# heliaxdev/kzg-setup-powersoftau

Measured on NVIDIA B200. Metric: G1+G2 points/sec parse+decompress+subgroup-check+ark re-encode (2^21 compressed G1 + 2^21 compressed G2 per step), higher is better.
Workload: dtype u32 limbs (12x32-bit Montgomery, IMAD.WIDE carry chains)

## Files before the change

### kzg_setup_powersoftau_b200/csrc/capi.cu

```cuda
#include <cuda_runtime.h>
#include <stdint.h>
#include <stdio.h>
#include <string.h>

#include <chrono>
#include <string>
#include <vector>

#include "../../include/ptau_b200.h"
#include <future>

#include "context.h"
#include "kernels.h"

using ptau::GpuSlot;
using ptau::kBufs;
using ptau::kMaxGpus;

namespace {

constexpr size_t kEdgePoints = 148 * 2 * 128;

#define CUDA_TRY(ctx, expr)                                                          \
  do {                                                                               \
// ... 320 lines not shown
        npts = rem < chunk ? rem : chunk;
      else if (rem > 2 * kEdgePoints)
        npts = rem - kEdgePoints;
      else
        npts = rem < chunk ? rem : chunk;
      if (r.issued >= kBufs) {
        CUDA_TRY(ctx, cudaEventSynchronize(s.ev_k1[b]));
        float ms = 0;
        CUDA_TRY(ctx, cudaEventElapsedTime(&ms, s.ev_k0[b], s.ev_k1[b]));
        tm.kernel_ms[g] += ms;
      }
      const uint8_t* src = (const uint8_t*)in + r.next * (size_t)ri;
      uint8_t* dst = out ? (uint8_t*)out + r.next * (size_t)ro : nullptr;
      CUDA_TRY(ctx, cudaMemcpyAsync(s.d_in[b], src, npts * ri, cudaMemcpyHostToDevice, s.stream[b]));
      CUDA_TRY(ctx, cudaEventRecord(s.ev_k0[b], s.stream[b]));
      CUDA_TRY(ctx, ptau::launch_convert(group, in_fmt, out_fmt, s.d_in[b], s.d_out[b], npts, checks, r.next,
                                         s.d_status, s.stream[b]));
      CUDA_TRY(ctx, cudaEventRecord(s.ev_k1[b], s.stream[b]));
      if (out) {
        CUDA_TRY(ctx, cudaMemcpyAsync(dst, s.d_out[b], npts * ro, cudaMemcpyDeviceToHost, s.stream[b]));
        tm.d2h_bytes[g] += npts * ro;
      }
      tm.h2d_bytes[g] += npts * ri;
      tm.kernel_launches++;
      r.next += npts;
      r.issued++;
      more = true;
    }
  }
  unsigned long long status = PTAU_STATUS_NONE;
  for (int g = 0; g < G; g++) {
    GpuSlot& s = ctx->gpu[g];
    CUDA_TRY(ctx, cudaSetDevice(s.device));
    CUDA_TRY(ctx, cudaEventRecord(s.ev_last, s.stream[1]));
    CUDA_TRY(ctx, cudaStreamWaitEvent(s.stream[0], s.ev_last, 0));
    unsigned long long st = PTAU_STATUS_NONE;
    CUDA_TRY(ctx, cudaMemcpyAsync(&st, s.d_status, sizeof(st), cudaMemcpyDeviceToHost, s.stream[0]));
    CUDA_TRY(ctx, cudaEventRecord(s.ev_last, s.stream[0]));
    CUDA_TRY(ctx, cudaStreamSynchronize(s.stream[0]));
    CUDA_TRY(ctx, cudaStreamSynchronize(s.stream[1]));
    if (st < status) status = st;
    float ms = 0;
    CUDA_TRY(ctx, cudaEventElapsedTime(&ms, s.ev_first, s.ev_last));
    tm.gpu_ms[g] = ms;
    int pending = rg[g].issued < kBufs ? rg[g].issued : kBufs;
    for (int b = 0; b < pending; b++) {
      float k = 0;
// ... 671 lines not shown
```

### kzg_setup_powersoftau_b200/csrc/consts.inc

```
PTAU_HD Fq k_b1_mont() {
  const uint32_t c[12] = {0x000cfff3u, 0xaa270000u, 0xfc34000au, 0x53cc0032u, 0x6b0a807fu, 0x478fe97au, 0xe6ba24d7u, 0xb1d37ebeu, 0xbf78ab2fu, 0x8ec9733bu, 0x3d83de7eu, 0x09d64551u};
  Fq r;
#pragma unroll
  for (int i = 0; i < 12; i++) r.l[i] = c[i];
  return r;
}
PTAU_HD Fq k_beta_mont() {
  const uint32_t c[12] = {0x798a64e8u, 0x30f1361bu, 0x7ece5a2au, 0xf3b8ddabu, 0xc61577f7u, 0x16a8ca3au, 0x74fd029bu, 0xc26a2ff8u, 0x60701c6eu, 0x3636b766u, 0x241b6160u, 0x051ba4abu};
  Fq r;
#pragma unroll
  for (int i = 0; i < 12; i++) r.l[i] = c[i];
  return r;
}
PTAU_HD Fq k_psi_cx1_mont() {
  const uint32_t c[12] = {0x867545c3u, 0x890dc9e4u, 0x3285a5d5u, 0x2af32253u, 0x309b7e2cu, 0x50880866u, 0x7e881024u, 0xa20d1b8cu, 0xe2db9068u, 0x14e4f04fu, 0x1564853au, 0x14e56d3fu};
  Fq r;
#pragma unroll
  for (int i = 0; i < 12; i++) r.l[i] = c[i];
  return r;
}
PTAU_HD Fq k_psi_cy0_mont() {
  const uint32_t c[12] = {0xa55c9ad1u, 0x3e2f585du, 0x86c18183u, 0x4294213du, 0x8b623732u, 0x382844c8u, 0x19103e18u, 0x92ad2afdu, 0xac7cf0b9u, 0x1d794e4fu, 0x7d825ec8u, 0x0bd592fcu};
  Fq r;
#pragma unroll
// ... 85 lines not shown
  return r;
}
PTAU_HD Fq k_frob12_c0_mont() {
  const uint32_t c[12] = {0xb319d465u, 0x07089552u, 0xb50a8313u, 0xc6695f92u, 0xd117228fu, 0x97e83cccu, 0xb2dc29eeu, 0xa35baecau, 0x5daace4du, 0x1ce393eau, 0xb0fb66ebu, 0x08f2220fu};
  Fq r;
#pragma unroll
  for (int i = 0; i < 12; i++) r.l[i] = c[i];
  return r;
}
PTAU_HD Fq k_frob12_c1_mont() {
  const uint32_t c[12] = {0x4ce5d646u, 0xb2f66aadu, 0xfc497cecu, 0x5842a06bu, 0x2599d394u, 0xcf4895d4u, 0x40a8e8d0u, 0xc11b9cbau, 0xe5a0de89u, 0x2e3813cbu, 0x88847fafu, 0x110eefdau};
  Fq r;
#pragma unroll
  for (int i = 0; i < 12; i++) r.l[i] = c[i];
  return r;
}
PTAU_HD Fq k_pm1_half_plain() {
  const uint32_t c[12] = {0xffffd555u, 0xdcff7fffu, 0x58a9ffffu, 0x0f55ffffu, 0x7b587b12u, 0xb3986950u, 0x79c2895fu, 0xb23ba5c2u, 0x21a5d66bu, 0x258dd3dbu, 0x1cbff34du, 0x0d0088f5u};
  Fq r;
#pragma unroll
  for (int i = 0; i < 12; i++) r.l[i] = c[i];
  return r;
}
#define PTAU_P34_STEPS 80
#define PTAU_P34_CHAIN_INIT {0x4d, 0x91, 0x41, 0x7f, 0x45, 0x67, 0x6b, 0x4f, 0x4f, 0x6d, 0x6d, 0x69, 0x33, 0x7d, 0x4d, 0x6f, 0x5d, 0x49, 0x8d, 0x6b, 0x35, 0x33, 0x6d, 0x47, 0x33, 0x31, 0x67, 0x47, 0x59, 0x47, 0x89, 0x37, 0x57, 0x75, 0x79, 0x5b, 0x4f, 0x33, 0x57, 0x43, 0x8d, 0x55, 0x21, 0x9f, 0x5d, 0x33, 0x8f, 0x33, 0x79, 0x9f, 0x45, 0x5b, 0x4f, 0x4f, 0x4f, 0x37, 0x5b, 0x65, 0x59, 0x4f, 0x4f, 0x4f, 0x4f, 0x4d, 0x23, 0x6f, 0x4f, 0x5f, 0x4f, 0x4f, 0x4f, 0x4f, 0x4f, 0x4f, 0x4f, 0x35, 0x45, 0x45, 0x21, 0x10}
```

### kzg_setup_powersoftau_b200/csrc/kernels.cu

```cuda
#include <cuda_runtime.h>
#include <stdint.h>
#include <string.h>

#include <type_traits>

#include "kernels.h"
#include "point.cuh"
#include "msm.cuh"

namespace ptau {

#ifndef PTAU_BLOCK
#define PTAU_BLOCK 128
#endif
#ifndef PTAU_MINBLOCKS_G1
#define PTAU_MINBLOCKS_G1 2
#endif
#ifndef PTAU_MINBLOCKS_G2
#define PTAU_MINBLOCKS_G2 2
#endif
#ifndef PTAU_BLOCK_G1
#define PTAU_BLOCK_G1 PTAU_BLOCK
#endif
#ifndef PTAU_BLOCK_G2
// ... 49 lines not shown
  }
}

template <int BLK>
__device__ __forceinline__ void stage_out_flat(uint32_t* __restrict__ g, const uint32_t* sm, int nwords) {
  int nvec = nwords >> 2;
  uint4* g4 = reinterpret_cast<uint4*>(g);
  const uint4* s4 = reinterpret_cast<const uint4*>(sm);
  for (int i = threadIdx.x; i < nvec; i += BLK) g4[i] = s4[i];
  for (int i = (nvec << 2) + threadIdx.x; i < nwords; i += BLK) g[i] = sm[i];
}

template <int G, int INFMT, int OUTFMT, bool HEAVY>
constexpr int convert_smem_words() {
  constexpr int BLK = G == PTAU_G1 ? PTAU_BLOCK_G1 : PTAU_BLOCK_G2;
  constexpr int SIN = smem_stride(record_bytes(G, INFMT) / 4);
  constexpr int SOUT = smem_stride(record_bytes(G, OUTFMT) / 4);
  return BLK * (SIN > SOUT ? SIN : SOUT) + ((G == PTAU_G2 && HEAVY) ? BLK * PTAU_PARK_WORDS : 0);
}

#ifndef PTAU_MINBLOCKS_LIGHT
#define PTAU_MINBLOCKS_LIGHT 2
#endif
template <int G, int INFMT, int OUTFMT, bool HEAVY>
__global__ void __launch_bounds__((G == PTAU_G1 ? PTAU_BLOCK_G1 : PTAU_BLOCK_G2),
                                  (!HEAVY ? PTAU_MINBLOCKS_LIGHT : G == PTAU_G1 ? PTAU_MINBLOCKS_G1 : PTAU_MINBLOCKS_G2))
    convert_kernel(const uint32_t* __restrict__ in, uint32_t* __restrict__ out, uint64_t n, uint32_t checks,
                   uint64_t base_index, unsigned long long* __restrict__ status) {
  constexpr int BLK = G == PTAU_G1 ? PTAU_BLOCK_G1 : PTAU_BLOCK_G2;
  constexpr int WIN = record_bytes(G, INFMT) / 4;
  constexpr int WOUT = record_bytes(G, OUTFMT) / 4;
  constexpr int SIN = smem_stride(WIN), SOUT = smem_stride(WOUT);
  constexpr int SMAX = SIN > SOUT ? SIN : SOUT;
  extern __shared__ __align__(16) uint32_t sm[];

  const uint64_t rec0 = (uint64_t)blockIdx.x * BLK;
  const int nrec = (int)((n - rec0) < (uint64_t)BLK ? (n - rec0) : (uint64_t)BLK);
  const int tid = threadIdx.x;

  stage_in<BLK, WIN, SIN>(in + rec0 * WIN, sm, nrec);
  __syncthreads();

  uint32_t win[WIN];
  if (tid < nrec) {
    if (WIN % 4 == 0) {
      const uint4* s4 = reinterpret_cast<const uint4*>(sm + tid * SIN);
#pragma unroll
      for (int j = 0; j < WIN / 4; j++) {
        uint4 v = s4[j];
        win[4 * j] = v.x;
        win[4 * j + 1] = v.y;
        win[4 * j + 2] = v.z;
        win[4 * j + 3] = v.w;
      }
    } else {
      const uint2* s2 = reinterpret_cast<const uint2*>(sm + tid * SIN);
#pragma unroll
      for (int j = 0; j < WIN / 2; j++) {
        uint2 v = s2[j];
        win[2 * j] = v.x;
        win[2 * j + 1] = v.y;
      }
    }
  }
  __syncthreads();

  if (tid < nrec) {
    uint32_t st;
    if (G == PTAU_G2 && HEAVY) {
      Park<BLK> pk;
      pk.base = (uint32_t)__cvta_generic_to_shared(sm + BLK * SMAX + tid);
      st = g2_process<INFMT, HEAVY, BLK>(win, OUTFMT, sm + tid * SOUT, checks, pk);
    } else {
      uint32_t wout[WOUT];
      if (G == PTAU_G2) {
        Park<BLK> pk;
        pk.base = 0;
        st = g2_process<INFMT, HEAVY, BLK>(win, OUTFMT, wout, checks, pk);
      } else {
        st = g1_process<INFMT, HEAVY>(win, OUTFMT, wout, checks);
      }
      if (WOUT % 4 == 0) {
        uint4* s4 = reinterpret_cast<uint4*>(sm + tid * SOUT);
#pragma unroll
        for (int j = 0; j < WOUT / 4; j++) s4[j] = make_uint4(wout[4 * j], wout[4 * j + 1], wout[4 * j + 2], wout[4 * j + 3]);
      } else {
        uint2* s2 = reinterpret_cast<uint2*>(sm + tid * SOUT);
#pragma unroll
        for (int j = 0; j < WOUT / 2; j++) s2[j] = make_uint2(wout[2 * j], wout[2 * j + 1]);
      }
    }
    if (st != PTAU_OK) atomicMin(status, (unsigned long long)(((base_index + rec0 + tid) << 8) | st));
  }
  __syncthreads();
  stage_out<BLK, WOUT, SOUT>(out + rec0 * WOUT, sm, nrec);
}

template <int G, int INFMT, int OUTFMT, bool HEAVY>
static cudaError_t launch_inst(const void* d_in, void* d_out, uint64_t n, uint32_t checks, uint64_t base_index,
                               unsigned long long* d_status, cudaStream_t stream) {
  constexpr int BLK = G == PTAU_G1 ? PTAU_BLOCK_G1 : PTAU_BLOCK_G2;
  constexpr int SMEM = convert_smem_words<G, INFMT, OUTFMT, HEAVY>() * 4;
  auto kern = convert_kernel<G, INFMT, OUTFMT, HEAVY>;
  if (SMEM > 48 * 1024) {
    cudaError_t e = cudaFuncSetAttribute(kern, cudaFuncAttributeMaxDynamicSharedMemorySize, SMEM);
    if (e != cudaSuccess) return e;
  }
  unsigned grid = (unsigned)((n + BLK - 1) / BLK);
  kern<<<grid, BLK, SMEM, stream>>>((const uint32_t*)d_in, (uint32_t*)d_out, n, checks, base_index, d_status);
  return cudaGetLastError();
}

template <int G, int INFMT, int OUTFMT>
static cudaError_t launch_one(const void* d_in, void* d_out, uint64_t n, uint32_t checks, uint64_t base_index,
                              unsigned long long* d_status, cudaStream_t stream) {
  if (n == 0) return cudaSuccess;
  const bool light = INFMT == PTAU_FMT_ZCASH_COMPRESSED
                         ? !(checks & PTAU_CHECK_SUBGROUP)
                         : !(checks & (PTAU_CHECK_ON_CURVE | PTAU_CHECK_SUBGROUP));
  if (light) return launch_inst<G, INFMT, OUTFMT, false>(d_in, d_out, n, checks, base_index, d_status, stream);
  return launch_inst<G, INFMT, OUTFMT, true>(d_in, d_out, n, checks, base_index, d_status, stream);
}

template <int G, int INFMT>
static cudaError_t launch_in(int out_fmt, const void* d_in, void* d_out, uint64_t n, uint32_t checks,
                             uint64_t base_index, unsigned long long* d_status, cudaStream_t stream) {
  switch (out_fmt) {
    case PTAU_FMT_ZCASH_UNCOMPRESSED:
      return launch_one<G, INFMT, PTAU_FMT_ZCASH_UNCOMPRESSED>(d_in, d_out, n, checks, base_index, d_status, stream);
    case PTAU_FMT_ARK_UNCOMPRESSED:
      return launch_one<G, INFMT, PTAU_FMT_ARK_UNCOMPRESSED>(d_in, d_out, n, checks, base_index, d_status, stream);
    case PTAU_FMT_ARK_MONT_LIMBS:
      return launch_one<G, INFMT, PTAU_FMT_ARK_MONT_LIMBS>(d_in, d_out, n, checks, base_index, d_status, stream);
  }
  return cudaErrorInvalidValue;
}

template <int G>
static cudaError_t launch_g(int in_fmt, int out_fmt, const void* d_in, void* d_out, uint64_t n, uint32_t checks,
                            uint64_t base_index, unsigned long long* d_status, cudaStream_t stream) {
  switch (in_fmt) {
    case PTAU_FMT_ZCASH_UNCOMPRESSED:
      return launch_in<G, PTAU_FMT_ZCASH_UNCOMPRESSED>(out_fmt, d_in, d_out, n, checks, base_index, d_status, stream);
    case PTAU_FMT_ZCASH_COMPRESSED:
// ... 899 lines not shown
```

### kzg_setup_powersoftau_b200/csrc/kernels.h

```cpp
#pragma once
#include <cuda_runtime.h>
#include <stdint.h>

namespace ptau {

struct MsmGeom;

cudaError_t launch_convert(int group, int in_fmt, int out_fmt, const void* d_in, void* d_out, uint64_t n,
                           uint32_t checks, uint64_t base_index, unsigned long long* d_status,
                           cudaStream_t stream);

cudaError_t launch_generate(int group, int fmt, const uint32_t* d_scalars, void* d_out, uint64_t n,
                            cudaStream_t stream);

cudaError_t launch_generate_win(int group, int fmt, const uint32_t* s0_mont, const uint32_t (*pw_mont)[8],
                                const uint32_t* d_tbl, void* d_out, uint64_t first, uint64_t n, cudaStream_t stream);

struct MsmPlan {
  int c, W, a, lgL;
  uint32_t NB;
  uint64_t buckets, segments;
  uint64_t off_counts, off_offsets, off_cursor, off_entries, off_buckets, off_segments, off_wsum, off_order, scratch_bytes;
};
void msm_g1_plan(uint64_t n, MsmPlan* plan);
cudaError_t launch_msm_g1(const void* d_pts, const void* d_scalars, uint64_t n, void* d_scratch, void* d_out,
                          int* launches, cudaStream_t stream);
void msm_g2_plan(uint64_t n, MsmPlan* plan);
cudaError_t launch_msm_g2(const void* d_pts, const void* d_scalars, uint64_t n, void* d_scratch, void* d_out,
                          int* launches, cudaStream_t stream);
cudaError_t launch_msm_g2_sums(const uint32_t* pts, const uint32_t* entries, const uint32_t* offsets, const uint32_t* order,
                               uint32_t m, uint32_t* buckets, const MsmGeom& g, uint32_t nseg, uint32_t* segs, uint32_t* wsum,
                               uint32_t* out, cudaStream_t stream);

// ... 17 lines not shown
```

### kzg_setup_powersoftau_b200/csrc/point.cuh

```cuda
#pragma once
#include "curve.cuh"
#include "../../include/ptau_b200.h"

namespace ptau {

PTAU_HD uint32_t bswap32(uint32_t v) {
#ifdef __CUDA_ARCH__
  return __byte_perm(v, 0, 0x0123);
#else
  return (v >> 24) | ((v >> 8) & 0xff00u) | ((v << 8) & 0xff0000u) | (v << 24);
#endif
}

PTAU_HD Fq fq_from_be_words(const uint32_t* w) {
  Fq r;
#pragma unroll
  for (int j = 0; j < 12; j++) r.l[j] = bswap32(w[11 - j]);
  return r;
}
PTAU_HD void fq_to_be_words(const Fq& a, uint32_t* w) {
#pragma unroll
  for (int j = 0; j < 12; j++) w[11 - j] = bswap32(a.l[j]);
}
PTAU_HD Fq fq_from_le_words(const uint32_t* w) {
  Fq r;
#pragma unroll
  for (int j = 0; j < 12; j++) r.l[j] = w[j];
  return r;
}
PTAU_HD void fq_to_le_words(const Fq& a, uint32_t* w) {
#pragma unroll
  for (int j = 0; j < 12; j++) w[j] = a.l[j];
}

#ifdef __CUDACC__
__constant__ uint8_t K_P34_CHAIN_D[PTAU_P34_STEPS] = PTAU_P34_CHAIN_INIT;
#endif
static const uint8_t K_P34_CHAIN_H[PTAU_P34_STEPS] = PTAU_P34_CHAIN_INIT;

PTAU_HD_NOINLINE Fq fq_pow_p34(const Fq& a) {
#ifdef __CUDA_ARCH__
  const uint8_t* chain = K_P34_CHAIN_D;
#else
  const uint8_t* chain = K_P34_CHAIN_H;
#endif
  Fq tbl[8];
  tbl[0] = a;
  Fq a2 = fq_sqr(a);
#pragma unroll 1
  for (int i = 1; i < 8; i++) tbl[i] = fq_mul(tbl[i - 1], a2);
  Fq acc = tbl[(chain[0] & 15) >> 1];
#pragma unroll 1
  for (int s = 1; s < PTAU_P34_STEPS; s++) {
    int c = chain[s];
    int n = c >> 4;
#if defined(__CUDA_ARCH__) && !defined(PTAU_POW_CALLS)
#pragma unroll 1
    for (int k = 0; k < n; k++) acc = fq_sqr_inl(acc);
#else
#pragma unroll 1
    for (int k = 0; k < n; k++) acc = fq_sqr(acc);
#endif
    if (c & 15) acc = fq_mul(acc, tbl[(c & 15) >> 1]);
  }
  return acc;
}

PTAU_HD Fq fq_sqrt(const Fq& a, bool& ok) {
  Fq s = fq_mul(fq_pow_p34(a), a);
  ok = fq_eq(fq_sqr(s), a);
  return s;
}

PTAU_HD_NOINLINE Fq2 fq2_sqrt(const Fq2& a, bool& ok) {
  Fq n = fq_add(fq_sqr(a.c0), fq_sqr(a.c1));
  Fq s = fq_mul(fq_pow_p34(n), n);
  Fq half = k_half_mont();
  Fq d = fq_mul(fq_add(a.c0, s), half);
  if (fq_is_zero(d)) d = fq_mul(fq_sub(a.c0, s), half);
  Fq t = fq_pow_p34(d);
  Fq x0 = fq_mul(d, t);
  Fq chi = fq_mul(x0, t);
  Fq w = fq_mul(fq_mul(a.c1, t), half);
  bool qr = fq_eq(chi, fq_one()) || fq_is_zero(d);
  Fq2 r;
  Fq nx0 = fq_neg(x0);
// ... 8 lines not shown

PTAU_HD bool fq_plain_is_largest(const Fq& yp) { return fq_gt_plain(yp, k_pm1_half_plain()); }

PTAU_HD Fq fq_plain_neg(const Fq& a) {
  const uint32_t pl[12] = PTAU_P_LIMBS;
  Fq r;
  uint32_t bf = 0;
  bool z = fq_is_zero(a);
#pragma unroll
  for (int i = 0; i < 12; i++) {
    uint64_t t = (uint64_t)pl[i] - a.l[i] - bf;
    bf = (uint32_t)(t >> 63);
    r.l[i] = z ? 0u : (uint32_t)t;
  }
  return r;
}

PTAU_HD constexpr int record_bytes(int group, int fmt) {
  return fmt == PTAU_FMT_ZCASH_COMPRESSED    ? (group == PTAU_G1 ? 48 : 96)
         : fmt == PTAU_FMT_ARK_MONT_LIMBS    ? (group == PTAU_G1 ? 104 : 200)
                                             : (group == PTAU_G1 ? 96 : 192);
}

template <int INFMT, bool HEAVY = true>
PTAU_HD uint32_t g1_process(const uint32_t* in, int out_fmt, uint32_t* out, uint32_t checks) {
  if (!HEAVY) checks &= PTAU_CHECK_REJECT_INFINITY;
  Fq xp, yp, xm, ym;
  uint32_t st = PTAU_OK;
  bool inf = false;
  bool have_mont = false;

  if (INFMT == PTAU_FMT_ZCASH_COMPRESSED) {
    xp = fq_from_be_words(in);
    uint32_t fl = xp.l[11] >> 29;
    xp.l[11] &= 0x1fffffffu;
    bool greatest = fl & 1u;
    yp = fq_zero();
    if (!(fl & 4u)) {
      st = PTAU_BAD_FLAGS;
    } else if (fl & 2u) {
      if ((fl & 1u) || !fq_is_zero(xp)) st = PTAU_BAD_FLAGS;
      inf = true;
      yp.l[0] = 1;
    } else if (fq_plain_ge_p(xp)) {
      st = PTAU_BAD_NON_CANONICAL;
    }
    if (st == PTAU_OK && !inf) {
      xm = fq_to_mont(xp);
      Fq rhs = fq_add(fq_mul(fq_sqr(xm), xm), k_b1_mont());
      bool ok;
      ym = fq_sqrt(rhs, ok);
      if (!ok) st = PTAU_BAD_NOT_ON_CURVE;
      yp = fq_from_mont(ym);
      if (fq_plain_is_largest(yp) != greatest) {
        ym = fq_neg(ym);
        yp = fq_plain_neg(yp);
      }
      have_mont = true;
    }
  } else if (INFMT == PTAU_FMT_ARK_MONT_LIMBS) {
    xm = fq_from_le_words(in);
    ym = fq_from_le_words(in + 12);
    inf = (in[24] & 0xffu) != 0;
    if (fq_plain_ge_p(xm) || fq_plain_ge_p(ym)) {
      st = PTAU_BAD_NON_CANONICAL;
      xm = fq_zero();
      ym = fq_zero();
    }
    have_mont = true;
    xp = fq_from_mont(xm);
    yp = fq_from_mont(ym);
    if (HEAVY && st == PTAU_OK && !inf && (checks & PTAU_CHECK_ON_CURVE) && !g1_on_curve(xm, ym)) st = PTAU_BAD_NOT_ON_CURVE;
  } else {
    if (INFMT == PTAU_FMT_ZCASH_UNCOMPRESSED) {
      xp = fq_from_be_words(in);
      yp = fq_from_be_words(in + 12);
    } else {
      xp = fq_from_le_words(in);
      yp = fq_from_le_words(in + 12);
    }
// ... 31 lines not shown
      out[0] = 0x40u;
    } else {
      fq_to_be_words(xp, out);
      fq_to_be_words(yp, out + 12);
    }
  } else {
    if (st == PTAU_OK && !have_mont) {
      xm = fq_to_mont(xp);
      ym = fq_to_mont(yp);
      have_mont = true;
    }
    if (!have_mont) {
      xm = fq_zero();
      ym = fq_zero();
    }
    fq_to_le_words(xm, out);
    fq_to_le_words(ym, out + 12);
    out[24] = inf ? 1u : 0u;
    out[25] = 0;
  }
  return st;
}

template <int INFMT, bool HEAVY, int PSTRIDE>
PTAU_HD uint32_t g2_process(const uint32_t* in, int out_fmt, uint32_t* out, uint32_t checks, Park<PSTRIDE> pk) {
  if (!HEAVY) checks &= PTAU_CHECK_REJECT_INFINITY;
  Fq2 xp, yp, xm, ym;
  uint32_t st = PTAU_OK;
  bool inf = false;
  bool have_mont = false;
  bool off_curve = false;

  if (INFMT == PTAU_FMT_ZCASH_COMPRESSED) {
    xp.c1 = fq_from_be_words(in);
    xp.c0 = fq_from_be_words(in + 12);
    uint32_t fl = xp.c1.l[11] >> 29;
    xp.c1.l[11] &= 0x1fffffffu;
    bool greatest = fl & 1u;
    yp = fq2_zero();
    if (!(fl & 4u)) {
      st = PTAU_BAD_FLAGS;
    } else if (fl & 2u) {
      if ((fl & 1u) || !fq2_is_zero(xp)) st = PTAU_BAD_FLAGS;
      inf = true;
      yp.c0.l[0] = 1;
    } else if (fq_plain_ge_p(xp.c1) || fq_plain_ge_p(xp.c0)) {
      st = PTAU_BAD_NON_CANONICAL;
    }
    if (st == PTAU_OK && !inf) {
      xm.c0 = fq_to_mont(xp.c0);
      xm.c1 = fq_to_mont(xp.c1);
      Fq2 b;
      b.c0 = k_b1_mont();
      b.c1 = b.c0;
      Fq2 rhs = fq2_add(fq2_mul(fq2_sqr(xm), xm), b);
      bool ok;
      ym = fq2_sqrt(rhs, ok);
      if (!ok) st = PTAU_BAD_NOT_ON_CURVE;
      yp.c0 = fq_from_mont(ym.c0);
      yp.c1 = fq_from_mont(ym.c1);
      bool largest = fq_is_zero(yp.c1) ? fq_plain_is_largest(yp.c0) : fq_plain_is_largest(yp.c1);
      if (largest != greatest) {
        ym = fq2_neg(ym);
        yp.c0 = fq_plain_neg(yp.c0);
        yp.c1 = fq_plain_neg(yp.c1);
      }
      have_mont = true;
    }
  } else if (INFMT == PTAU_FMT_ARK_MONT_LIMBS) {
    xm.c0 = fq_from_le_words(in);
    xm.c1 = fq_from_le_words(in + 12);
    ym.c0 = fq_from_le_words(in + 24);
    ym.c1 = fq_from_le_words(in + 36);
    inf = (in[48] & 0xffu) != 0;
    if (fq_plain_ge_p(xm.c0) || fq_plain_ge_p(xm.c1) || fq_plain_ge_p(ym.c0) || fq_plain_ge_p(ym.c1)) {
      st = PTAU_BAD_NON_CANONICAL;
      xm = fq2_zero();
      ym = fq2_zero();
    }
    have_mont = true;
    xp.c0 = fq_from_mont(xm.c0);
    xp.c1 = fq_from_mont(xm.c1);
    yp.c0 = fq_from_mont(ym.c0);
    yp.c1 = fq_from_mont(ym.c1);
    if (HEAVY && st == PTAU_OK && !inf && (checks & (PTAU_CHECK_ON_CURVE | PTAU_CHECK_SUBGROUP)) && !g2_on_curve(xm, ym)) {
      if (checks & PTAU_CHECK_ON_CURVE) {
        st = PTAU_BAD_NOT_ON_CURVE;
      } else {
        off_curve = true;
// ... 64 lines not shown
    if (st == PTAU_OK && !have_mont) {
      xm.c0 = fq_to_mont(xp.c0);
      xm.c1 = fq_to_mont(xp.c1);
      ym.c0 = fq_to_mont(yp.c0);
      ym.c1 = fq_to_mont(yp.c1);
      have_mont = true;
    }
    if (!have_mont) {
      xm = fq2_zero();
      ym = fq2_zero();
    }
    fq_to_le_words(xm.c0, out);
    fq_to_le_words(xm.c1, out + 12);
    fq_to_le_words(ym.c0, out + 24);
    fq_to_le_words(ym.c1, out + 36);
    out[48] = inf ? 1u : 0u;
    out[49] = 0;
  }
  if (ladder && !g2_in_subgroup(pk)) st = PTAU_BAD_NOT_IN_SUBGROUP;
  return st;
}

#ifndef __CUDA_ARCH__
template <int INFMT, bool HEAVY = true>
inline uint32_t g2_process(const uint32_t* in, int out_fmt, uint32_t* out, uint32_t checks) {
  uint32_t file[PTAU_PARK_WORDS];
  Park<1> pk;
  pk.p = file;
  return g2_process<INFMT, HEAVY, 1>(in, out_fmt, out, checks, pk);
}
#endif

}
```

### kzg_setup_powersoftau_b200/csrc/verify.cu

```cuda
#include <cuda_runtime.h>
#include <stdint.h>
#include <string.h>
#include <sys/random.h>

#include <chrono>
#include <string>
#include <vector>

#include "../../include/ptau_b200.h"
#include "blake2b.h"
#include "context.h"
#include "curve.cuh"
#include "kernels.h"

namespace ptau {

constexpr uint64_t kSlabChunks = 16;

struct B2Key {
  uint64_t h[8];
};

__global__ void __launch_bounds__(256) ratio_coeff_kernel(B2Key key, uint32_t k, uint64_t first, uint64_t n,
                                                          uint32_t* __restrict__ out) {
// ... 287 lines not shown
      VTRY(cudaMalloc(&x.d_sc, max_pts * 32 + 16));
      VTRY(cudaMalloc(&x.d_scratch, scratch));
      VTRY(cudaMalloc((void**)&x.d_parts, (size_t)x.parts * 256));
    }
    VTRY(cudaMemcpyAsync(x.d_status, none_v.data(), nsec * 8, cudaMemcpyHostToDevice, s.stream[0]));
    VTRY(cudaStreamSynchronize(s.stream[0]));
  }
  uint64_t launches = 0, h2d = 0;

  {
    GpuSlot& s = ctx->gpu[0];
    VTRY(cudaSetDevice(s.device));
    VTRY(cudaMalloc(&run.d_keys, kKeyWords * 4));
    VTRY(cudaMalloc(&run.d_keys_in, 256));
    VTRY(cudaMalloc((void**)&run.d_key_status, 8));
    VTRY(cudaMemsetAsync(run.d_keys, 0, kKeyWords * 4, s.stream[0]));
    for (const KeyPoint& kp : keys) {
      const Sec& sc = secs[kp.sec];
      const int ri = rec_bytes(sc.group, fmt);
      uint32_t* dst = (uint32_t*)run.d_keys + (sc.group == PTAU_G1 ? kp.slot * 32 : K1_N * 32 + kp.slot * 64);
      VTRY(cudaMemcpyAsync(run.d_keys_in, sc.data + kp.index * ri, ri, cudaMemcpyHostToDevice, s.stream[0]));
      VTRY(launch_convert(sc.group, fmt, PTAU_FMT_ARK_MONT_LIMBS, run.d_keys_in, dst, 1, PTAU_CHECKS_STRICT, 0,
                          run.d_key_status, s.stream[0]));
      launches++;
    }
  }

  std::vector<size_t> next(G, 0);
  std::vector<std::vector<int>> per_gpu(G);
  for (int j = 0; j < (int)jobs.size(); j++) per_gpu[jobs[j].gpu].push_back(j);
  bool more = true;
  while (more) {
    more = false;
    for (int g = 0; g < G; g++) {
      if (next[g] >= per_gpu[g].size()) continue;
      more = true;
      const Job& jb = jobs[per_gpu[g][next[g]++]];
      const Piece& pc = pieces[jb.piece];
      const Sec& sc = secs[pc.sec];
      const int ri = rec_bytes(sc.group, fmt), rb = sc.group == PTAU_G1 ? 104 : 200;
      GpuSlot& s = ctx->gpu[g];
      GpuWork& x = run.w[g];
      VTRY(cudaSetDevice(s.device));
      VTRY(cudaEventRecord(x.ev, s.stream[0]));
      VTRY(cudaStreamWaitEvent(s.stream[1], x.ev, 0));
      int c = 0;
      for (uint64_t o = jb.a; o < jb.b; o += chunk, c++) {
        const uint64_t m = jb.b - o < chunk ? jb.b - o : chunk;
        const uint64_t idx = pc.first + o;
        cudaStream_t st = s.stream[c & 1];
        VTRY(cudaMemcpyAsync(x.d_in[c & 1], sc.data + idx * ri, m * ri, cudaMemcpyHostToDevice, st));
        VTRY(launch_convert(sc.group, fmt, PTAU_FMT_ARK_MONT_LIMBS, x.d_in[c & 1], (uint8_t*)x.d_rec + (o - jb.a) * rb, m,
                            PTAU_CHECKS_STRICT, idx, x.d_status + pc.sec, st));
        launches++;
        h2d += m * ri;
      }
      VTRY(cudaEventRecord(x.ev, s.stream[1]));
      VTRY(cudaStreamWaitEvent(s.stream[0], x.ev, 0));
      if (jb.part < 0) continue;
      const uint64_t np = jb.b - 1 - jb.a;
      ratio_coeff_kernel<<<(unsigned)((np + 255) / 256), 256, 0, s.stream[0]>>>(key, (uint32_t)pc.rel, jb.a, np,
                                                                                  (uint32_t*)x.d_sc);
      VTRY(cudaGetLastError());
      auto msm = sc.group == PTAU_G1 ? launch_msm_g1 : launch_msm_g2;
      int nl = 0;
      VTRY(msm(x.d_rec, x.d_sc, np, x.d_scratch, x.d_parts + (size_t)jb.part * 256, &nl, s.stream[0]));
      launches += nl + 1;
      VTRY(msm((uint8_t*)x.d_rec + rb, x.d_sc, np, x.d_scratch, x.d_parts + (size_t)(jb.part + 1) * 256, &nl, s.stream[0]));
      launches += nl;
    }
  }

  std::vector<std::vector<uint8_t>> parts(G);
  unsigned long long st_min[8];
  for (int i = 0; i < nsec; i++) st_min[i] = none;
  for (int g = 0; g < G; g++) {
    GpuSlot& s = ctx->gpu[g];
// ... 100 lines not shown
```

Baseline: 18.15 million.

## Split compressed-point sqrt into separate kernel and use windowed p34 addition chain

Strict compressed conversion now runs as two kernels. A dedicated sqrt kernel with its own launch bounds decompresses y and writes it into the output buffer, and the heavy convert kernel then reads y back instead of recomputing the square root. Separately, the p-3/4 exponentiation uses a larger precomputed table with a sliding-window chain, which cuts the number of steps and multiplications. The split is meant to free register pressure so each kernel gets better occupancy, at the cost of an extra launch and a y round-trip through global memory.

Result: faster. 18.63 million, median of 6 (+2.6%).

```diff
diff --git a/kzg_setup_powersoftau_b200/csrc/capi.cu b/kzg_setup_powersoftau_b200/csrc/capi.cu
--- a/kzg_setup_powersoftau_b200/csrc/capi.cu
+++ b/kzg_setup_powersoftau_b200/csrc/capi.cu
@@ -366,7 +366,7 @@
         tm.d2h_bytes[g] += npts * ro;
       }
       tm.h2d_bytes[g] += npts * ri;
-      tm.kernel_launches++;
+      tm.kernel_launches += ptau::convert_launches(in_fmt, checks);
       r.next += npts;
       r.issued++;
       more = true;
diff --git a/kzg_setup_powersoftau_b200/csrc/consts.inc b/kzg_setup_powersoftau_b200/csrc/consts.inc
--- a/kzg_setup_powersoftau_b200/csrc/consts.inc
+++ b/kzg_setup_powersoftau_b200/csrc/consts.inc
@@ -131,5 +131,7 @@
   for (int i = 0; i < 12; i++) r.l[i] = c[i];
   return r;
 }
-#define PTAU_P34_STEPS 80
-#define PTAU_P34_CHAIN_INIT {0x4d, 0x91, 0x41, 0x7f, 0x45, 0x67, 0x6b, 0x4f, 0x4f, 0x6d, 0x6d, 0x69, 0x33, 0x7d, 0x4d, 0x6f, 0x5d, 0x49, 0x8d, 0x6b, 0x35, 0x33, 0x6d, 0x47, 0x33, 0x31, 0x67, 0x47, 0x59, 0x47, 0x89, 0x37, 0x57, 0x75, 0x79, 0x5b, 0x4f, 0x33, 0x57, 0x43, 0x8d, 0x55, 0x21, 0x9f, 0x5d, 0x33, 0x8f, 0x33, 0x79, 0x9f, 0x45, 0x5b, 0x4f, 0x4f, 0x4f, 0x37, 0x5b, 0x65, 0x59, 0x4f, 0x4f, 0x4f, 0x4f, 0x4d, 0x23, 0x6f, 0x4f, 0x5f, 0x4f, 0x4f, 0x4f, 0x4f, 0x4f, 0x4f, 0x4f, 0x35, 0x45, 0x45, 0x21, 0x10}
+#define PTAU_P34_TBL 18
+#define PTAU_P34_TBL_INIT {0xff0100u, 0x010000u, 0x010002u, 0x010003u, 0x010004u, 0x010005u, 0x010006u, 0x010007u, 0x010008u, 0x010009u, 0x01000au, 0x01000bu, 0x01000cu, 0x01000du, 0x01000eu, 0x01000fu, 0x000110u}
+#define PTAU_P34_STEPS 64
+#define PTAU_P34_CHAIN_INIT {0x0007, 0x0d09, 0x0708, 0x0403, 0x0604, 0x070c, 0x0611, 0x050a, 0x060a, 0x0505, 0x0606, 0x080e, 0x0303, 0x0608, 0x060e, 0x0300, 0x0807, 0x070c, 0x0506, 0x0607, 0x060f, 0x0405, 0x080f, 0x0407, 0x070c, 0x090a, 0x050d, 0x0202, 0x0703, 0x0705, 0x060c, 0x050f, 0x050a, 0x050a, 0x0807, 0x070b, 0x0908, 0x0507, 0x0302, 0x0808, 0x0302, 0x0705, 0x0908, 0x060b, 0x0711, 0x0611, 0x0510, 0x0506, 0x080b, 0x0811, 0x0611, 0x0611, 0x050c, 0x0811, 0x050e, 0x0611, 0x0611, 0x0611, 0x0611, 0x0611, 0x050b, 0x060b, 0x0200, 0x01ff}
diff --git a/kzg_setup_powersoftau_b200/csrc/kernels.cu b/kzg_setup_powersoftau_b200/csrc/kernels.cu
--- a/kzg_setup_powersoftau_b200/csrc/kernels.cu
+++ b/kzg_setup_powersoftau_b200/csrc/kernels.cu
@@ -95,11 +95,68 @@
 #ifndef PTAU_MINBLOCKS_LIGHT
 #define PTAU_MINBLOCKS_LIGHT 2
 #endif
-template <int G, int INFMT, int OUTFMT, bool HEAVY>
+template <int G>
+__host__ __device__ constexpr int yin_words() { return G == PTAU_G1 ? 12 : 24; }
+
+template <int W, int S>
+__device__ __forceinline__ void gather_record(const uint32_t* sm, uint32_t* w) {
+  if (W % 4 == 0) {
+    const uint4* s4 = reinterpret_cast<const uint4*>(sm + threadIdx.x * S);
+#pragma unroll
+    for (int j = 0; j < W / 4; j++) {
+      uint4 v = s4[j];
+      w[4 * j] = v.x;
+      w[4 * j + 1] = v.y;
+      w[4 * j + 2] = v.z;
+      w[4 * j + 3] = v.w;
+    }
+  } else {
+    const uint2* s2 = reinterpret_cast<const uint2*>(sm + threadIdx.x * S);
+#pragma unroll
+    for (int j = 0; j < W / 2; j++) {
+      uint2 v = s2[j];
+      w[2 * j] = v.x;
+      w[2 * j + 1] = v.y;
+    }
+  }
+}
+
+#ifndef PTAU_MINBLOCKS_SQRT
+#define PTAU_MINBLOCKS_SQRT 3
+#endif
+template <int G, int WOUT>
+__global__ void __launch_bounds__(PTAU_BLOCK, PTAU_MINBLOCKS_SQRT)
+    sqrt_kernel(const uint32_t* __restrict__ in, uint32_t* __restrict__ out, uint64_t n) {
+  constexpr int BLK = PTAU_BLOCK;
+  constexpr int WIN = record_bytes(G, PTAU_FMT_ZCASH_COMPRESSED) / 4;
+  constexpr int SIN = smem_stride(WIN);
+  constexpr int YW = yin_words<G>();
+  static_assert(WOUT >= YW, "y must fit the output slot");
+  __shared__ __align__(16) uint32_t sm[BLK * SIN];
+
+  const uint64_t rec0 = (uint64_t)blockIdx.x * BLK;
+  const int nrec = (int)((n - rec0) < (uint64_t)BLK ? (n - rec0) : (uint64_t)BLK);
+  const int tid = threadIdx.x;
+  stage_in<BLK, WIN, SIN>(in + rec0 * WIN, sm, nrec);
+  __syncthreads();
+  if (tid >= nrec) return;
+  uint32_t win[WIN], y[YW];
+  gather_record<WIN, SIN>(sm, win);
+  if (G == PTAU_G1)
+    g1_sqrt_stage(win, y);
+  else
+    g2_sqrt_stage(win, y);
+  uint2* o2 = reinterpret_cast<uint2*>(out + (rec0 + tid) * WOUT);
+#pragma unroll
+  for (int j = 0; j < YW / 2; j++) o2[j] = make_uint2(y[2 * j], y[2 * j + 1]);
+}
+
+template <int G, int INFMT, int OUTFMT, bool HEAVY, bool YIN>
 __global__ void __launch_bounds__((G == PTAU_G1 ? PTAU_BLOCK_G1 : PTAU_BLOCK_G2),
                                   (!HEAVY ? PTAU_MINBLOCKS_LIGHT : G == PTAU_G1 ? PTAU_MINBLOCKS_G1 : PTAU_MINBLOCKS_G2))
     convert_kernel(const uint32_t* __restrict__ in, uint32_t* __restrict__ out, uint64_t n, uint32_t checks,
                    uint64_t base_index, unsigned long long* __restrict__ status) {
+  static_assert(!YIN || (INFMT == PTAU_FMT_ZCASH_COMPRESSED && HEAVY), "YIN: strict compressed conversion only");
   constexpr int BLK = G == PTAU_G1 ? PTAU_BLOCK_G1 : PTAU_BLOCK_G2;
   constexpr int WIN = record_bytes(G, INFMT) / 4;
   constexpr int WOUT = record_bytes(G, OUTFMT) / 4;
@@ -114,25 +171,17 @@
   stage_in<BLK, WIN, SIN>(in + rec0 * WIN, sm, nrec);
   __syncthreads();
 
-  uint32_t win[WIN];
+  constexpr int YW = YIN ? yin_words<G>() : 2;
+  uint32_t win[WIN], yin[YW];
   if (tid < nrec) {
-    if (WIN % 4 == 0) {
-      const uint4* s4 = reinterpret_cast<const uint4*>(sm + tid * SIN);
-#pragma unroll
-      for (int j = 0; j < WIN / 4; j++) {
-        uint4 v = s4[j];
-        win[4 * j] = v.x;
-        win[4 * j + 1] = v.y;
-        win[4 * j + 2] = v.z;
-        win[4 * j + 3] = v.w;
-      }
-    } else {
-      const uint2* s2 = reinterpret_cast<const uint2*>(sm + tid * SIN);
-#pragma unroll
-      for (int j = 0; j < WIN / 2; j++) {
-        uint2 v = s2[j];
-        win[2 * j] = v.x;
-        win[2 * j + 1] = v.y;
+    gather_record<WIN, SIN>(sm, win);
+    if (YIN) {
+      const uint2* y2 = reinterpret_cast<const uint2*>(out + (rec0 + tid) * WOUT);
+#pragma unroll
+      for (int j = 0; j < YW / 2; j++) {
+        uint2 v = y2[j];
+        yin[2 * j] = v.x;
+        yin[2 * j + 1] = v.y;
       }
     }
   }
@@ -143,15 +192,15 @@
     if (G == PTAU_G2 && HEAVY) {
       Park<BLK> pk;
       pk.base = (uint32_t)__cvta_generic_to_shared(sm + BLK * SMAX + tid);
-      st = g2_process<INFMT, HEAVY, BLK>(win, OUTFMT, sm + tid * SOUT, checks, pk);
+      st = g2_process<INFMT, HEAVY, BLK, YIN>(win, OUTFMT, sm + tid * SOUT, checks, pk, yin);
     } else {
       uint32_t wout[WOUT];
       if (G == PTAU_G2) {
         Park<BLK> pk;
         pk.base = 0;
-        st = g2_process<INFMT, HEAVY, BLK>(win, OUTFMT, wout, checks, pk);
+        st = g2_process<INFMT, HEAVY, BLK, YIN>(win, OUTFMT, wout, checks, pk, yin);
       } else {
-        st = g1_process<INFMT, HEAVY>(win, OUTFMT, wout, checks);
+        st = g1_process<INFMT, HEAVY, YIN>(win, OUTFMT, wout, checks, yin);
       }
       if (WOUT % 4 == 0) {
         uint4* s4 = reinterpret_cast<uint4*>(sm + tid * SOUT);
@@ -169,12 +218,12 @@
   stage_out<BLK, WOUT, SOUT>(out + rec0 * WOUT, sm, nrec);
 }
 
-template <int G, int INFMT, int OUTFMT, bool HEAVY>
+template <int G, int INFMT, int OUTFMT, bool HEAVY, bool YIN = false>
 static cudaError_t launch_inst(const void* d_in, void* d_out, uint64_t n, uint32_t checks, uint64_t base_index,
                                unsigned long long* d_status, cudaStream_t stream) {
   constexpr int BLK = G == PTAU_G1 ? PTAU_BLOCK_G1 : PTAU_BLOCK_G2;
   constexpr int SMEM = convert_smem_words<G, INFMT, OUTFMT, HEAVY>() * 4;
-  auto kern = convert_kernel<G, INFMT, OUTFMT, HEAVY>;
+  auto kern = convert_kernel<G, INFMT, OUTFMT, HEAVY, YIN>;
   if (SMEM > 48 * 1024) {
     cudaError_t e = cudaFuncSetAttribute(kern, cudaFuncAttributeMaxDynamicSharedMemorySize, SMEM);
     if (e != cudaSuccess) return e;
@@ -182,17 +231,33 @@
   unsigned grid = (unsigned)((n + BLK - 1) / BLK);
   kern<<<grid, BLK, SMEM, stream>>>((const uint32_t*)d_in, (uint32_t*)d_out, n, checks, base_index, d_status);
   return cudaGetLastError();
+}
+
+static bool convert_is_light(int in_fmt, uint32_t checks) {
+  return in_fmt == PTAU_FMT_ZCASH_COMPRESSED ? !(checks & PTAU_CHECK_SUBGROUP)
+                                             : !(checks & (PTAU_CHECK_ON_CURVE | PTAU_CHECK_SUBGROUP));
+}
+
+int convert_launches(int in_fmt, uint32_t checks) {
+  return (in_fmt == PTAU_FMT_ZCASH_COMPRESSED && !convert_is_light(in_fmt, checks)) ? 2 : 1;
 }
 
 template <int G, int INFMT, int OUTFMT>
 static cudaError_t launch_one(const void* d_in, void* d_out, uint64_t n, uint32_t checks, uint64_t base_index,
                               unsigned long long* d_status, cudaStream_t stream) {
   if (n == 0) return cudaSuccess;
-  const bool light = INFMT == PTAU_FMT_ZCASH_COMPRESSED
-                         ? !(checks & PTAU_CHECK_SUBGROUP)
-                         : !(checks & (PTAU_CHECK_ON_CURVE | PTAU_CHECK_SUBGROUP));
-  if (light) return launch_inst<G, INFMT, OUTFMT, false>(d_in, d_out, n, checks, base_index, d_status, stream);
-  return launch_inst<G, INFMT, OUTFMT, true>(d_in, d_out, n, checks, base_index, d_status, stream);
+  if (convert_is_light(INFMT, checks))
+    return launch_inst<G, INFMT, OUTFMT, false>(d_in, d_out, n, checks, base_index, d_status, stream);
+  if constexpr (INFMT == PTAU_FMT_ZCASH_COMPRESSED) {
+    constexpr int WOUT = record_bytes(G, OUTFMT) / 4;
+    sqrt_kernel<G, WOUT><<<(unsigned)((n + PTAU_BLOCK - 1) / PTAU_BLOCK), PTAU_BLOCK, 0, stream>>>(
+        (const uint32_t*)d_in, (uint32_t*)d_out, n);
+    cudaError_t e = cudaGetLastError();
+    if (e != cudaSuccess) return e;
+    return launch_inst<G, INFMT, OUTFMT, true, true>(d_in, d_out, n, checks, base_index, d_status, stream);
+  } else {
+    return launch_inst<G, INFMT, OUTFMT, true>(d_in, d_out, n, checks, base_index, d_status, stream);
+  }
 }
 
 template <int G, int INFMT>
diff --git a/kzg_setup_powersoftau_b200/csrc/kernels.h b/kzg_setup_powersoftau_b200/csrc/kernels.h
--- a/kzg_setup_powersoftau_b200/csrc/kernels.h
+++ b/kzg_setup_powersoftau_b200/csrc/kernels.h
@@ -9,6 +9,7 @@
 cudaError_t launch_convert(int group, int in_fmt, int out_fmt, const void* d_in, void* d_out, uint64_t n,
                            uint32_t checks, uint64_t base_index, unsigned long long* d_status,
                            cudaStream_t stream);
+int convert_launches(int in_fmt, uint32_t checks);
 
 cudaError_t launch_generate(int group, int fmt, const uint32_t* d_scalars, void* d_out, uint64_t n,
                             cudaStream_t stream);
diff --git a/kzg_setup_powersoftau_b200/csrc/point.cuh b/kzg_setup_powersoftau_b200/csrc/point.cuh
--- a/kzg_setup_powersoftau_b200/csrc/point.cuh
+++ b/kzg_setup_powersoftau_b200/csrc/point.cuh
@@ -34,26 +34,36 @@
 }
 
 #ifdef __CUDACC__
-__constant__ uint8_t K_P34_CHAIN_D[PTAU_P34_STEPS] = PTAU_P34_CHAIN_INIT;
-#endif
-static const uint8_t K_P34_CHAIN_H[PTAU_P34_STEPS] = PTAU_P34_CHAIN_INIT;
+__constant__ uint32_t K_P34_TBL_D[PTAU_P34_TBL - 1] = PTAU_P34_TBL_INIT;
+__constant__ uint16_t K_P34_CHAIN_D[PTAU_P34_STEPS] = PTAU_P34_CHAIN_INIT;
+#endif
+static const uint32_t K_P34_TBL_H[PTAU_P34_TBL - 1] = PTAU_P34_TBL_INIT;
+static const uint16_t K_P34_CHAIN_H[PTAU_P34_STEPS] = PTAU_P34_CHAIN_INIT;
 
 PTAU_HD_NOINLINE Fq fq_pow_p34(const Fq& a) {
 #ifdef __CUDA_ARCH__
-  const uint8_t* chain = K_P34_CHAIN_D;
+  const uint32_t* prog = K_P34_TBL_D;
+  const uint16_t* chain = K_P34_CHAIN_D;
 #else
-  const uint8_t* chain = K_P34_CHAIN_H;
-#endif
-  Fq tbl[8];
+  const uint32_t* prog = K_P34_TBL_H;
+  const uint16_t* chain = K_P34_CHAIN_H;
+#endif
+  Fq tbl[PTAU_P34_TBL];
   tbl[0] = a;
-  Fq a2 = fq_sqr(a);
 #pragma unroll 1
-  for (int i = 1; i < 8; i++) tbl[i] = fq_mul(tbl[i - 1], a2);
-  Fq acc = tbl[(chain[0] & 15) >> 1];
+  for (int k = 1; k < PTAU_P34_TBL; k++) {
+    uint32_t c = prog[k - 1];
+    Fq t = tbl[c & 0xff];
+#pragma unroll 1
+    for (int i = 0; i < (int)((c >> 8) & 0xff); i++) t = fq_sqr(t);
+    if ((c >> 16) != 0xff) t = fq_mul(t, tbl[c >> 16]);
+    tbl[k] = t;
+  }
+  Fq acc = tbl[chain[0] & 0xff];
 #pragma unroll 1
   for (int s = 1; s < PTAU_P34_STEPS; s++) {
     int c = chain[s];
-    int n = c >> 4;
+    int n = c >> 8;
 #if defined(__CUDA_ARCH__) && !defined(PTAU_POW_CALLS)
 #pragma unroll 1
     for (int k = 0; k < n; k++) acc = fq_sqr_inl(acc);
@@ -61,7 +71,7 @@
 #pragma unroll 1
     for (int k = 0; k < n; k++) acc = fq_sqr(acc);
 #endif
-    if (c & 15) acc = fq_mul(acc, tbl[(c & 15) >> 1]);
+    if ((c & 0xff) != 0xff) acc = fq_mul(acc, tbl[c & 0xff]);
   }
   return acc;
 }
@@ -116,8 +126,57 @@
                                              : (group == PTAU_G1 ? 96 : 192);
 }
 
-template <int INFMT, bool HEAVY = true>
-PTAU_HD uint32_t g1_process(const uint32_t* in, int out_fmt, uint32_t* out, uint32_t checks) {
+constexpr uint32_t PTAU_YIN_NOT_SQUARE = 0x80000000u;
+
+PTAU_HD uint32_t g1_parse_compressed(const uint32_t* in, Fq& xp, bool& greatest, bool& inf) {
+  xp = fq_from_be_words(in);
+  uint32_t fl = xp.l[11] >> 29;
+  xp.l[11] &= 0x1fffffffu;
+  greatest = fl & 1u;
+  inf = false;
+  if (!(fl & 4u)) return PTAU_BAD_FLAGS;
+  if (fl & 2u) {
+    inf = true;
+    return ((fl & 1u) || !fq_is_zero(xp)) ? PTAU_BAD_FLAGS : PTAU_OK;
+  }
+  return fq_plain_ge_p(xp) ? PTAU_BAD_NON_CANONICAL : PTAU_OK;
+}
+
+PTAU_HD Fq g1_decompress_y(const Fq& xm, bool greatest, bool& ok, Fq& yp) {
+  Fq rhs = fq_add(fq_mul(fq_sqr(xm), xm), k_b1_mont());
+  Fq ym = fq_sqrt(rhs, ok);
+  yp = fq_from_mont(ym);
+  if (fq_plain_is_largest(yp) != greatest) {
+    ym = fq_neg(ym);
+    yp = fq_plain_neg(yp);
+  }
+  return ym;
+}
+
+PTAU_HD void g1_sqrt_stage(const uint32_t* in, uint32_t* yout) {
+  Fq xp, ym = fq_zero();
+  bool greatest, inf, ok = true;
+  if (g1_parse_compressed(in, xp, greatest, inf) == PTAU_OK && !inf) {
+    Fq yp;
+    ym = g1_decompress_y(fq_to_mont(xp), greatest, ok, yp);
+  }
+  if (!ok) ym.l[11] |= PTAU_YIN_NOT_SQUARE;
+  fq_to_le_words(ym, yout);
+}
+
+template <int INFMT, bool HEAVY = true, bool YIN = false>
+PTAU_HD uint32_t g1_process(const uint32_t* in, int out_fmt, uint32_t* out, uint32_t checks,
+                            const uint32_t* yin = nullptr) {
+#ifndef __CUDA_ARCH__
+  if constexpr (INFMT == PTAU_FMT_ZCASH_COMPRESSED && HEAVY && !YIN) {
+    if (checks & PTAU_CHECK_SUBGROUP) {
+      uint32_t y[12];
+      g1_sqrt_stage(in, out);
+      for (int i = 0; i < 12; i++) y[i] = out[i];
+      return g1_process<INFMT, true, true>(in, out_fmt, out, checks, y);
+    }
+  }
+#endif
   if (!HEAVY) checks &= PTAU_CHECK_REJECT_INFINITY;
   Fq xp, yp, xm, ym;
   uint32_t st = PTAU_OK;
@@ -125,31 +184,22 @@
   bool have_mont = false;
 
   if (INFMT == PTAU_FMT_ZCASH_COMPRESSED) {
-    xp = fq_from_be_words(in);
-    uint32_t fl = xp.l[11] >> 29;
-    xp.l[11] &= 0x1fffffffu;
-    bool greatest = fl & 1u;
+    bool greatest;
+    st = g1_parse_compressed(in, xp, greatest, inf);
     yp = fq_zero();
-    if (!(fl & 4u)) {
-      st = PTAU_BAD_FLAGS;
-    } else if (fl & 2u) {
-      if ((fl & 1u) || !fq_is_zero(xp)) st = PTAU_BAD_FLAGS;
-      inf = true;
-      yp.l[0] = 1;
-    } else if (fq_plain_ge_p(xp)) {
-      st = PTAU_BAD_NON_CANONICAL;
-    }
+    if (inf) yp.l[0] = 1;
     if (st == PTAU_OK && !inf) {
       xm = fq_to_mont(xp);
-      Fq rhs = fq_add(fq_mul(fq_sqr(xm), xm), k_b1_mont());
       bool ok;
-      ym = fq_sqrt(rhs, ok);
+      if (YIN) {
+        ym = fq_from_le_words(yin);
+        ok = !(ym.l[11] & PTAU_YIN_NOT_SQUARE);
+        ym.l[11] &= ~PTAU_YIN_NOT_SQUARE;
+        yp = fq_from_mont(ym);
+      } else {
+        ym = g1_decompress_y(xm, greatest, ok, yp);
+      }
       if (!ok) st = PTAU_BAD_NOT_ON_CURVE;
-      yp = fq_from_mont(ym);
-      if (fq_plain_is_largest(yp) != greatest) {
-        ym = fq_neg(ym);
-        yp = fq_plain_neg(yp);
-      }
       have_mont = true;
     }
   } else if (INFMT == PTAU_FMT_ARK_MONT_LIMBS) {
@@ -227,8 +277,55 @@
   return st;
 }
 
-template <int INFMT, bool HEAVY, int PSTRIDE>
-PTAU_HD uint32_t g2_process(const uint32_t* in, int out_fmt, uint32_t* out, uint32_t checks, Park<PSTRIDE> pk) {
+PTAU_HD uint32_t g2_parse_compressed(const uint32_t* in, Fq2& xp, bool& greatest, bool& inf) {
+  xp.c1 = fq_from_be_words(in);
+  xp.c0 = fq_from_be_words(in + 12);
+  uint32_t fl = xp.c1.l[11] >> 29;
+  xp.c1.l[11] &= 0x1fffffffu;
+  greatest = fl & 1u;
+  inf = false;
+  if (!(fl & 4u)) return PTAU_BAD_FLAGS;
+  if (fl & 2u) {
+    inf = true;
+    return ((fl & 1u) || !fq2_is_zero(xp)) ? PTAU_BAD_FLAGS : PTAU_OK;
+  }
+  return (fq_plain_ge_p(xp.c1) || fq_plain_ge_p(xp.c0)) ? PTAU_BAD_NON_CANONICAL : PTAU_OK;
+}
+
+PTAU_HD Fq2 g2_decompress_y(const Fq2& xm, bool greatest, bool& ok, Fq2& yp) {
+  Fq2 b;
+  b.c0 = k_b1_mont();
+  b.c1 = b.c0;
+  Fq2 rhs = fq2_add(fq2_mul(fq2_sqr(xm), xm), b);
+  Fq2 ym = fq2_sqrt(rhs, ok);
+  yp.c0 = fq_from_mont(ym.c0);
+  yp.c1 = fq_from_mont(ym.c1);
+  bool largest = fq_is_zero(yp.c1) ? fq_plain_is_largest(yp.c0) : fq_plain_is_largest(yp.c1);
+  if (largest != greatest) {
+    ym = fq2_neg(ym);
+    yp.c0 = fq_plain_neg(yp.c0);
+    yp.c1 = fq_plain_neg(yp.c1);
+  }
+  return ym;
+}
+
+PTAU_HD void g2_sqrt_stage(const uint32_t* in, uint32_t* yout) {
+  Fq2 xp, ym = fq2_zero();
+  bool greatest, inf, ok = true;
+  if (g2_parse_compressed(in, xp, greatest, inf) == PTAU_OK && !inf) {
+    Fq2 xm, yp;
+    xm.c0 = fq_to_mont(xp.c0);
+    xm.c1 = fq_to_mont(xp.c1);
+    ym = g2_decompress_y(xm, greatest, ok, yp);
+  }
+  if (!ok) ym.c1.l[11] |= PTAU_YIN_NOT_SQUARE;
+  fq_to_le_words(ym.c0, yout);
+  fq_to_le_words(ym.c1, yout + 12);
+}
+
+template <int INFMT, bool HEAVY, int PSTRIDE, bool YIN = false>
+PTAU_HD uint32_t g2_process(const uint32_t* in, int out_fmt, uint32_t* out, uint32_t checks, Park<PSTRIDE> pk,
+                            const uint32_t* yin = nullptr) {
   if (!HEAVY) checks &= PTAU_CHECK_REJECT_INFINITY;
   Fq2 xp, yp, xm, ym;
   uint32_t st = PTAU_OK;
@@ -237,39 +334,25 @@
   bool off_curve = false;
 
   if (INFMT == PTAU_FMT_ZCASH_COMPRESSED) {
-    xp.c1 = fq_from_be_words(in);
-    xp.c0 = fq_from_be_words(in + 12);
-    uint32_t fl = xp.c1.l[11] >> 29;
-    xp.c1.l[11] &= 0x1fffffffu;
-    bool greatest = fl & 1u;
+    bool greatest;
+    st = g2_parse_compressed(in, xp, greatest, inf);
     yp = fq2_zero();
-    if (!(fl & 4u)) {
-      st = PTAU_BAD_FLAGS;
-    } else if (fl & 2u) {
-      if ((fl & 1u) || !fq2_is_zero(xp)) st = PTAU_BAD_FLAGS;
-      inf = true;
-      yp.c0.l[0] = 1;
-    } else if (fq_plain_ge_p(xp.c1) || fq_plain_ge_p(xp.c0)) {
-      st = PTAU_BAD_NON_CANONICAL;
-    }
+    if (inf) yp.c0.l[0] = 1;
     if (st == PTAU_OK && !inf) {
       xm.c0 = fq_to_mont(xp.c0);
       xm.c1 = fq_to_mont(xp.c1);
-      Fq2 b;
-      b.c0 = k_b1_mont();
-      b.c1 = b.c0;
-      Fq2 rhs = fq2_add(fq2_mul(fq2_sqr(xm), xm), b);
       bool ok;
-      ym = fq2_sqrt(rhs, ok);
+      if (YIN) {
+        ym.c0 = fq_from_le_words(yin);
+        ym.c1 = fq_from_le_words(yin + 12);
+        ok = !(ym.c1.l[11] & PTAU_YIN_NOT_SQUARE);
+        ym.c1.l[11] &= ~PTAU_YIN_NOT_SQUARE;
+        yp.c0 = fq_from_mont(ym.c0);
+        yp.c1 = fq_from_mont(ym.c1);
+      } else {
+        ym = g2_decompress_y(xm, greatest, ok, yp);
+      }
       if (!ok) st = PTAU_BAD_NOT_ON_CURVE;
-      yp.c0 = fq_from_mont(ym.c0);
-      yp.c1 = fq_from_mont(ym.c1);
-      bool largest = fq_is_zero(yp.c1) ? fq_plain_is_largest(yp.c0) : fq_plain_is_largest(yp.c1);
-      if (largest != greatest) {
-        ym = fq2_neg(ym);
-        yp.c0 = fq_plain_neg(yp.c0);
-        yp.c1 = fq_plain_neg(yp.c1);
-      }
       have_mont = true;
     }
   } else if (INFMT == PTAU_FMT_ARK_MONT_LIMBS) {
@@ -380,13 +463,22 @@
 }
 
 #ifndef __CUDA_ARCH__
-template <int INFMT, bool HEAVY = true>
-inline uint32_t g2_process(const uint32_t* in, int out_fmt, uint32_t* out, uint32_t checks) {
+template <int INFMT, bool HEAVY = true, bool YIN = false>
+inline uint32_t g2_process(const uint32_t* in, int out_fmt, uint32_t* out, uint32_t checks,
+                           const uint32_t* yin = nullptr) {
   uint32_t file[PTAU_PARK_WORDS];
   Park<1> pk;
   pk.p = file;
-  return g2_process<INFMT, HEAVY, 1>(in, out_fmt, out, checks, pk);
-}
-#endif
-
-}
+  if constexpr (INFMT == PTAU_FMT_ZCASH_COMPRESSED && HEAVY && !YIN) {
+    if (checks & PTAU_CHECK_SUBGROUP) {
+      uint32_t y[24];
+      g2_sqrt_stage(in, out);
+      for (int i = 0; i < 24; i++) y[i] = out[i];
+      return g2_process<INFMT, true, 1, true>(in, out_fmt, out, checks, pk, y);
+    }
+  }
+  return g2_process<INFMT, HEAVY, 1, YIN>(in, out_fmt, out, checks, pk, yin);
+}
+#endif
+
+}
diff --git a/kzg_setup_powersoftau_b200/csrc/verify.cu b/kzg_setup_powersoftau_b200/csrc/verify.cu
--- a/kzg_setup_powersoftau_b200/csrc/verify.cu
+++ b/kzg_setup_powersoftau_b200/csrc/verify.cu
@@ -333,7 +333,7 @@
       VTRY(cudaMemcpyAsync(run.d_keys_in, sc.data + kp.index * ri, ri, cudaMemcpyHostToDevice, s.stream[0]));
       VTRY(launch_convert(sc.group, fmt, PTAU_FMT_ARK_MONT_LIMBS, run.d_keys_in, dst, 1, PTAU_CHECKS_STRICT, 0,
                           run.d_key_status, s.stream[0]));
-      launches++;
+      launches += convert_launches(fmt, PTAU_CHECKS_STRICT);
     }
   }
 
@@ -363,7 +363,7 @@
         VTRY(cudaMemcpyAsync(x.d_in[c & 1], sc.data + idx * ri, m * ri, cudaMemcpyHostToDevice, st));
         VTRY(launch_convert(sc.group, fmt, PTAU_FMT_ARK_MONT_LIMBS, x.d_in[c & 1], (uint8_t*)x.d_rec + (o - jb.a) * rb, m,
                             PTAU_CHECKS_STRICT, idx, x.d_status + pc.sec, st));
-        launches++;
+        launches += convert_launches(fmt, PTAU_CHECKS_STRICT);
         h2d += m * ri;
       }
       VTRY(cudaEventRecord(x.ev, s.stream[1]));
```
